# iamwangyabin/hardnetNas

Hardware: AMD Instinct MI355X
Metric: Mpatches/s (32×32→128-D) at 1/2/4/8 MI355X; HPatches FPR95 parity (higher is better)
Workload: dtype bf16x3; 1 GPU; Stock HardNet forward, 262144 synthetic 32x32 patches per GPU; model=hardnet, global_batch=262144, per_gpu_batch=262144, parallelism=dp1

## Files before the change

### hardnetnas_amd/csrc/hn_api.hip

```cpp
#include "hardnet_mi355x.h"
#include "hn_api_util.h"
#include "hn_internal.h"
#include "hn_pack.h"

#include <algorithm>
#include <atomic>
#include <cmath>
#include <cstdlib>
#include <cstring>
#include <map>
#include <mutex>
#include <string>
#include <utility>
#include <vector>

static thread_local std::string g_err;

static int env_int(const char* name, int dflt) {
  const char* e = std::getenv(name);
  return e ? std::atoi(e) : dflt;
}

void hn_read_knobs(HnKnobs* k) {
  *k = HnKnobs{};
// ... 2 lines not shown
  k->head_pf = env_int("HN_HEAD_PF", 1) != 0;
  k->fdl_valu = std::getenv("HN_FDL_VALU") != nullptr;
  k->naive_pw = std::getenv("HN_NAIVE_PW") != nullptr;
  k->naive_dw = std::getenv("HN_NAIVE_DW") != nullptr;
  k->no_skipfuse = std::getenv("HN_NO_SKIPFUSE") != nullptr;
  k->no_irfskip = std::getenv("HN_NO_IRFSKIP") != nullptr;
  k->pairdist_valu = std::getenv("HN_PAIRDIST_VALU") != nullptr;
  k->pairdist_reg = env_int("HN_PAIRDIST_REG", 0) != 0;
  k->pairdist_spread = env_int("HN_PAIRDIST_SPREAD", 1) != 0;
  k->front_fold = env_int("HN_FRONT_FOLD", 0) != 0;
  k->u8_apart = env_int("HN_U8_APART", 0) != 0;
  k->front_xch3 = env_int("HN_FRONT_XCH3", 0) != 0;
  k->no_mpfront = env_int("HN_NO_MPFRONT", 0) != 0;
  k->pipeline = env_int("HN_PIPELINE", 0) != 0;
  k->dyn_tiles = env_int("HN_STATIC_TILES", 0) != 0 ? 0 : env_int("HN_DYN_TILES", 3) & (kTilesConv3 | kTilesConv5);

  k->train_splitk = std::max(32, env_int("HN_TRAIN_SPLITK", 1024)) / 32 * 32;
  k->train_f32 = env_int("HN_TRAIN_F32", 17) & 255;
#ifdef HN_EXPERIMENTS
  k->c12_abl = env_int("HN_C12_ABL", 0) & 4095;
  k->c12w_pd = env_int("HN_C12W_PD", 11);
  k->dbg = env_int("HN_DEBUG", 0);
  k->head_abl = env_int("HN_HEAD_ABL", 0);
  k->w4_abl = env_int("HN_W4_ABL", 0);
  k->pairdist_abl = env_int("HN_PAIRDIST_ABL", 0);
  k->irf3 = env_int("HN_IRF3", 0) != 0;
#endif
}

static thread_local const HnKnobs* tl_knobs = nullptr;
// ... 286 lines not shown
    Folded f = fold(w, per, cout[l], nullptr, nullptr, mean, var, eps);
    int rc;
    if (l == 0) {
      std::vector<float> sw(9 * 32);
      for (int n = 0; n < 32; ++n)
        for (int t = 0; t < 9; ++t) sw[t * 32 + n] = f.w[n * 9 + t];
      if ((rc = m->upload(sw, &m->hd.stem_w))) return rc;
      if ((rc = m->upload(f.b, &m->hd.stem_b))) return rc;
      continue;
    }
    std::vector<uint16_t> pk = (l < 6) ? pack_conv3x3(f.w, cin[l], cout[l]) : pack_head(f.w, 128, 8);
    uint16_t* d = nullptr;
    if ((rc = m->upload(pk, &d))) return rc;
    m->hd.wpack[l] = d;
    if ((rc = m->upload(f.b, &m->hd.bias[l]))) return rc;
    if (l == 3 || l == 5) {
      uint16_t* c = nullptr;
      if ((rc = m->upload(pack_wino1(f.w, cin[l], cout[l]), &c))) return rc;
      m->hd.wino1[l] = c;
    }
#ifdef HN_EXPERIMENTS
    if (l == 3) {
      uint16_t* c = nullptr;
      if ((rc = m->upload(pack_wino4(f.w, cin[l], cout[l]), &c))) return rc;
      m->hd.wino4[l] = c;
    }
    if (l == 3 || l == 5) {
      uint16_t* c = nullptr;
      if ((rc = m->upload(pack_wino(f.w, cin[l], cout[l]), &c))) return rc;
      m->hd.wino[l] = c;
// ... 220 lines not shown
      if (*c >= '0' && *c <= '9') variant[i++] = *c - '0';
      else if (*c >= 'a' && *c <= 'z') variant[i++] = 10 + (*c - 'a');
  }
  hn_read_knobs(&m->knobs);
  if (m->knobs.head == 4 && !std::getenv("HN_CHUNK")) m->chunk = 65536;
  for (int l = 0; l < 6; ++l)
    if (!(m->conv[l] = hn_hardnet_conv_row(l, variant[l]))) {
      const std::string msg = "HN_VARIANT: tiling " + std::to_string(variant[l]) +
                              " is not available for layer " + std::to_string(l);
      delete m;
      return fail(HN_ERR_ARG, msg);
    }
  if (!hn_c12_cfg_ok(m->knobs.c12_cfg, m->knobs.c12_abl, m->knobs.c12w_pd)) {
    delete m;
    return fail(HN_ERR_ARG, "HN_C12_CFG / HN_C12_ABL / HN_C12W_PD: no such k_c12 build in this library");
  }
  if (m->knobs.head < 1 || m->knobs.head > 4) {
    delete m;
    return fail(HN_ERR_ARG, "HN_HEAD: head GEMM form must be 1, 2, 3 or 4");
  }
  (void)hipGetDevice(&m->device);
  Cursor cur{host_params, n_params};
  tl_f16_out_of_range = 0;
  rc = desc->kind == HN_KIND_HARDNET ? build_hardnet(m, cur)
       : desc->kind == HN_KIND_NAS    ? build_nas(m, cur)
                                      : build_fdl(m, cur);
  if (!rc && cur.i != n_params) rc = fail(HN_ERR_ARG, "host_params not fully consumed");
  if (!rc && tl_f16_out_of_range)
    rc = fail(HN_ERR_ARG, std::to_string(tl_f16_out_of_range) +
                              " BN-folded weights are outside the fp16 range of the fp16x3 kernels (|w| >= 65520 "
// ... 457 lines not shown
```

### hardnetnas_amd/csrc/hn_common.h

```cpp
#pragma once
#include <hip/hip_runtime.h>
#include <stdint.h>

typedef __bf16 bf16x8 __attribute__((ext_vector_type(8)));
typedef float f32x16 __attribute__((ext_vector_type(16)));
typedef float f32x4 __attribute__((ext_vector_type(4)));

#define HN_DEV __device__ __forceinline__

HN_DEV float relu0(float x) { return __builtin_bit_cast(float, __builtin_elementwise_max(__builtin_bit_cast(int, x), 0)); }
HN_DEV f32x4 relu4(f32x4 v) { return f32x4{relu0(v[0]), relu0(v[1]), relu0(v[2]), relu0(v[3])}; }

HN_DEV void split_bf16(float x, __bf16& hi, __bf16& lo) {
  hi = (__bf16)x;
  lo = (__bf16)(x - (float)hi);
}

typedef __bf16 bf16x4 __attribute__((ext_vector_type(4)));

HN_DEV void split8(const float4& a, const float4& b, uint4& hi, uint4& lo) {
  const float v[8] = {a.x, a.y, a.z, a.w, b.x, b.y, b.z, b.w};
  bf16x8 h, l;
#pragma unroll
  for (int j = 0; j < 8; ++j) {
// ... 46 lines not shown
                        f32x16 acc) {
  acc = __builtin_amdgcn_mfma_f32_32x32x16_f16(al, bh, acc, 0, 0, 0);
  acc = __builtin_amdgcn_mfma_f32_32x32x16_f16(ah, bl, acc, 0, 0, 0);
  acc = __builtin_amdgcn_mfma_f32_32x32x16_f16(ah, bh, acc, 0, 0, 0);
  return acc;
}

typedef float f32x4_t __attribute__((ext_vector_type(4)));
HN_DEV f32x4_t mfma3_f16_16(const f16x8& ah, const f16x8& al, const f16x8& bh, const f16x8& bl, f32x4_t acc) {
  acc = __builtin_amdgcn_mfma_f32_16x16x32_f16(al, bh, acc, 0, 0, 0);
  acc = __builtin_amdgcn_mfma_f32_16x16x32_f16(ah, bl, acc, 0, 0, 0);
  acc = __builtin_amdgcn_mfma_f32_16x16x32_f16(ah, bh, acc, 0, 0, 0);
  return acc;
}

HN_DEV int xcd_remap(int bid, int nblocks) {
  const int xcd = bid & 7, idx = bid >> 3;
  const int q = nblocks >> 3, r = nblocks & 7;
  return (xcd < r ? xcd * (q + 1) : r * (q + 1) + (xcd - r) * q) + idx;
}

HN_DEV float wave_sum(float v) {
#pragma unroll
  for (int o = 32; o > 0; o >>= 1) v += __shfl_xor(v, o, 64);
  return v;
}

HN_DEV float half_sum(float v) {
#pragma unroll
  for (int o = 16; o > 0; o >>= 1) v += __shfl_xor(v, o, 64);
// ... 3 lines not shown
```

### hardnetnas_amd/csrc/hn_hardnet.hip

```cpp
#include "hn_common.h"
#include "hn_internal.h"

#include <algorithm>
#include <cstdlib>

template <bool NORM>
__global__ __launch_bounds__(256) void k_stem(const float* __restrict__ in, float* __restrict__ out,
                                              const float* __restrict__ w,
                                              const float* __restrict__ b,
                                              float eps) {
  __shared__ float tile[34 * 34];
  __shared__ float red[8];
  const int t = threadIdx.x;
  const size_t p = blockIdx.x;
  const float4 v = reinterpret_cast<const float4*>(in + p * 1024)[t];
  for (int i = t; i < 34 * 34; i += 256) tile[i] = 0.f;
  float mean = 0.f, sd = 1.f;
  if (NORM) {
    float s = wave_sum(v.x + v.y + v.z + v.w);
    if ((t & 63) == 0) red[t >> 6] = s;
    __syncthreads();
    mean = (red[0] + red[1] + red[2] + red[3]) * (1.f / 1024.f);
    const float d0 = v.x - mean, d1 = v.y - mean, d2 = v.z - mean, d3 = v.w - mean;
    float q = wave_sum(d0 * d0 + d1 * d1 + d2 * d2 + d3 * d3);
// ... 633 lines not shown
  static constexpr int SCR = 32 * SROW * 4;
  static constexpr int OSTR = COUT * 4 + 16;
  static constexpr int OCH = B::BM * COUT / 4;
  static constexpr int OPT = OCH / PTHR;
  static constexpr int MB = PST ? (B::BM < BUF / OSTR ? B::BM : BUF / OSTR) : 0;
  static constexpr int XST = PST ? (B::BM - MB) * OSTR : 0;
  static constexpr int BIAS_OFF = 2 * BUF + (STEM ? NWP * PBUF : 0) + (CST ? NWC * SCR : 0);
  static constexpr int SMEM = BIAS_OFF + COUT * 4 + XST;
  static constexpr bool DEEP = !STEM && UPT <= 6;
  static_assert(SMEM <= 160 * 1024, "LDS");
  static_assert(!(STEM && CST), "the CST epilogue scratch starts where the STEM buffers live");
  static_assert(!PST || (!STEM && !CST && OCH % PTHR == 0), "PST");
};

template <int CIN, int COUT, int HIN, int S, int NP, int TR, int WM, int WN, bool STEM, int ABL = 0,
          int PX = 80, bool CST = false, bool PST = false>
__global__ __launch_bounds__((WM * WN + 4) * 64) void k_conv_ws(
    const float* __restrict__ in, float* __restrict__ out, const uint4* __restrict__ wp,
    const float* __restrict__ bias, int P, const float* __restrict__ stem_w,
    const float* __restrict__ stem_b, float eps, float relu_lo) {
  using C = WsCfg<CIN, COUT, HIN, S, NP, TR, WM, WN, STEM, PX, CST, PST>;
  static_assert(PX == 80 || !STEM, "the stem producer writes the 80-byte layout");
  extern __shared__ __attribute__((aligned(16))) char smem[];
  const int tid = threadIdx.x, lane = tid & 63;
  const int wave = __builtin_amdgcn_readfirstlane(tid >> 6);
  const bool producer = wave >= C::NWC;
  const int r = lane & 31, h = lane >> 5;
  const int nwg = gridDim.x, rb = xcd_remap(blockIdx.x, nwg);
  const int ntiles = (P + NP - 1) / NP * C::RT;
  const int per = (ntiles + nwg - 1) / nwg;
  const int t_begin = STEM ? rb * per : rb;
// ... 160 lines not shown
#pragma unroll
        for (int q = 0; q < 4; ++q) {
          bf16x4 oh, ol;
#pragma unroll
          for (int j = 0; j < 4; ++j) {
            const float v = inside ? fmaxf(c0[4 * q + j] + b16[4 * q + j], 0.f) : 0.f;
            oh[j] = (__bf16)v;
            ol[j] = (__bf16)(v - (float)oh[j]);
          }
          *reinterpret_cast<uint2*>(o + 16 * q) = __builtin_bit_cast(uint2, oh);
          *reinterpret_cast<uint2*>(o + C::PLANE + 16 * q) = __builtin_bit_cast(uint2, ol);
        }
      }
    }
  };

  if (producer) {
    if constexpr (STEM) {
      static_assert(CIN == 32 && HIN == 32 && S == 1 && NP == 1, "stem fusion is conv1-only");
      for (int i = lane; i < 34 * 34; i += 64) pt[i] = 0.f;
      stem_loads(0);
      stem_write(0, buf0);
    } else {
      produce_loads(0, pf);
      produce_write(buf0, pf);
      if (NS > 1) produce_loads(1, pf);
    }
  } else {
    for (int i = tid; i < COUT; i += C::NWC * 64) reinterpret_cast<float*>(smem + C::BIAS_OFF)[i] = bias[i];
  }
// ... 781 lines not shown

using Conv1s = Direct<32, 32, 32, 1, 1, 8, 4, 1, true>;
using Conv1 = Direct<32, 32, 32, 1, 1, 8, 4, 1, false>;
using Conv2 = Direct<32, 64, 32, 2, 1, 8, 2, 2, false>;
using Conv3 = Direct<64, 64, 16, 1, 1, 16, 2, 2, false>;
using Conv4 = Direct<64, 128, 16, 2, 1, 8, 1, 4, false>;
using Conv5 = Direct<128, 128, 8, 1, 2, 8, 1, 4, false>;
using Pipe5Cst = Pipe<128, 128, 8, 1, 2, 8, 1, 4, false, 0, true>;
using Ws1s = Ws<32, 32, 32, 1, 1, 4, 4, 1, true, 0, 80, false, false>;
using Ws1sT8 = Ws<32, 32, 32, 1, 1, 8, 4, 1, true, 0, 80, false, false>;
using Ws2 = Ws<32, 64, 32, 2, 1, 4, 2, 2, false, 0, 80, false, false>;
using Ws2T2 = Ws<32, 64, 32, 2, 1, 2, 1, 2, false, 0, 80, false, false>;
using Ws4Np2 = Ws<64, 128, 16, 2, 2, 8, 2, 2, false, 0, 64, false, false>;
using Ws4Pst = Ws<64, 128, 16, 2, 2, 8, 2, 2, false, 0, 64, false, true>;
using Ws3Cst = Ws<64, 64, 16, 1, 1, 16, 2, 2, false, 0, 80, true, false>;

constexpr HnConvRow kConvRows[] = {
    {0, 0, row<0, Conv1s>},
    {0, 5, row<0, Ws1s>},
    {0, 6, row<0, Ws1sT8>},
    {1, 0, row<1, Conv1>},
    {1, 5, row<1, Conv1>},
    {1, 6, row<1, Conv1>},
    {2, 0, row<2, Conv2>},
    {2, 5, row<2, Ws2>},
    {2, 6, row<2, Ws2T2>},
    {3, 0, row<3, Conv3>},
    {3, 16, row<3, Ws3Cst>},
    {4, 0, row<4, Conv4>},
    {4, 15, row<4, Ws4Np2>},
    {4, 18, row<4, Ws4Pst>},
    {5, 0, row<5, Conv5>},
    {5, 16, row<5, Pipe5Cst>},
#ifdef HN_EXPERIMENTS
    {0, 1, row<0, Direct<32, 32, 32, 1, 1, 4, 4, 1, true>>},
    {2, 1, row<2, Direct<32, 64, 32, 2, 1, 4, 2, 2, false>>},
    {3, 1, row<3, Direct<64, 64, 16, 1, 1, 8, 2, 2, false>>},
    {4, 1, row<4, Direct<64, 128, 16, 2, 1, 4, 1, 4, false>>},
    {5, 1, row<5, Direct<128, 128, 8, 1, 1, 8, 1, 4, false>>},
    {0, 2, row<0, Pipe<32, 32, 32, 1, 1, 4, 4, 1, true, 0, false>>},
    {0, 3, row<0, Pipe<32, 32, 32, 1, 1, 8, 4, 1, true, 0, false>>},
    {2, 2, row<2, Pipe<32, 64, 32, 2, 1, 2, 1, 2, false, 0, false>>},
    {2, 3, row<2, Pipe<32, 64, 32, 2, 1, 4, 2, 2, false, 0, false>>},
    {3, 2, row<3, Pipe<64, 64, 16, 1, 1, 8, 2, 2, false, 0, false>>},
    {3, 3, row<3, Pipe<64, 64, 16, 1, 1, 16, 2, 2, false, 0, false>>},
    {4, 2, row<4, Pipe<64, 128, 16, 2, 1, 4, 1, 4, false, 0, false>>},
// ... 144 lines not shown
```

### hardnetnas_amd/csrc/hn_internal.h

```cpp
#pragma once
#include <hip/hip_runtime.h>

#include <algorithm>
#include <type_traits>

#include "hardnet_mi355x.h"

struct HnKnobs {
  int c12_cfg = 15;
  int head = 4;
  bool head_pf = true;
  bool fdl_valu = false;
  bool naive_pw = false;
  bool naive_dw = false;
  bool no_skipfuse = false;
  bool no_irfskip = false;
  bool pairdist_valu = false;
  bool pairdist_reg = false;
  bool pairdist_spread = true;
  bool front_fold = false;
  bool u8_apart = false;
  bool front_xch3 = false;
  bool no_mpfront = false;
  bool pipeline = false;
  bool irf3 = false;
  int dyn_tiles = 3;
  int train_splitk = 1024;
  int train_f32 = 17;
  int c12w_pd = 11;
  int c12_abl = 0;
  int head_abl = 0;
  int w4_abl = 0;
  int pairdist_abl = 0;
  int dbg = 0;
};
void hn_read_knobs(HnKnobs* k);
const HnKnobs& hn_knobs();

constexpr int kTilesConv3 = 1, kTilesConv5 = 2;
constexpr int kTileLaunches = 32;
unsigned* hn_tile_counters(int kernel);

hipError_t hn_resident_blocks(const void* fn, int nthreads, int lds, int* resident);

struct HardnetDev {
  float* stem_w = nullptr;
  float* stem_b = nullptr;
  void* wpack[7] = {};
  float* bias[7] = {};
  void* c12_w1 = nullptr;
  void* c12_w2 = nullptr;
  void* c12_w1w = nullptr;
  void* wino[7] = {};
  void* wino1[7] = {};
  void* wino4[7] = {};
};
struct HnU8In {
  const uint8_t* in;
  int resize;
  int normalize;
  float mean, stdv;
};
hipError_t hn_launch_c12(const float* in, float* out, const HardnetDev& d, int P, float eps,
                         hipStream_t st, const HnU8In* u8 = nullptr);

hipError_t hn_launch_stem(const float* in, float* out, const float* w, const float* b, int P,
                          bool norm, float eps, hipStream_t st);
using HnConvLaunch = hipError_t (*)(const HardnetDev& d, const float* in, float* out, int P, float eps,
                                    hipStream_t st);
// ... 278 lines not shown
```

### hardnetnas_amd/csrc/hn_pack.h

```cpp
#pragma once
#include <cmath>
#include <cstddef>
#include <cstdint>
#include <cstring>
#include <vector>

namespace {

uint16_t f2bf(float x) {
  uint32_t u;
  std::memcpy(&u, &x, 4);
  u += 0x7FFFu + ((u >> 16) & 1u);
  return (uint16_t)(u >> 16);
}
float bf2f(uint16_t b) {
  uint32_t u = (uint32_t)b << 16;
  float f;
  std::memcpy(&f, &u, 4);
  return f;
}

struct Folded {
  std::vector<float> w, b;
};
// ... 25 lines not shown
          uint16_t* lo = &out[o + 64 * 8];
          for (int lane = 0; lane < 64; ++lane)
            for (int j = 0; j < 8; ++j) {
              const int n = nt * 32 + (lane & 31);
              const int c = cc * 32 + ks * 16 + (lane >> 5) * 8 + j;
              const float v = w[((size_t)n * cin + c) * 9 + tap];
              const uint16_t h = f2bf(v);
              hi[lane * 8 + j] = h;
              lo[lane * 8 + j] = f2bf(v - bf2f(h));
            }
          o += 2 * 64 * 8;
        }
  return out;
}

static thread_local long tl_f16_out_of_range = 0;
static void put_f16_split(float v, uint16_t* hi, uint16_t* lo) {
  const _Float16 hv = (_Float16)v;
  if (!std::isfinite((float)hv)) ++tl_f16_out_of_range;
  const _Float16 lv = (_Float16)(v - (float)hv);
  std::memcpy(hi, &hv, 2);
  std::memcpy(lo, &lv, 2);
}

static std::vector<uint16_t> pack_head(const std::vector<float>& w, int cin, int kk, bool f16 = false) {
  const int K = cin * kk * kk;
  std::vector<uint16_t> out((size_t)(K / 16) * 4 * 2 * 64 * 8);
  size_t o = 0;
  for (int ks = 0; ks < K / 16; ++ks)
    for (int nt = 0; nt < 4; ++nt) {
// ... 145 lines not shown
          for (int j = 0; j < 8; ++j) {
            const int n = nt * 32 + (lane & 31);
            const int c = cc * 32 + ks * 16 + (lane >> 5) * 8 + j;
            double u = 0;
            for (int t = 0; t < 3; ++t) u += G[xi][t] * (double)w[((size_t)n * cin + c) * 9 + ky * 3 + t];
            const float v = (float)(xi == 3 ? -u : u);
            const uint16_t hv = f2bf(v);
            hi[lane * 8 + j] = hv;
            lo[lane * 8 + j] = f2bf(v - bf2f(hv));
          }
        o += 2 * 64 * 8;
      }
  return out;
}

static std::vector<uint16_t> pack_wino4(const std::vector<float>& w, int cin, int cout) {
  static const double G[6][3] = {{4, 0, 0},
                                 {2.0 / 3, 2.0 / 3, 2.0 / 3},
                                 {2.0 / 3, -2.0 / 3, 2.0 / 3},
                                 {-8.0 / 3, -4.0 / 3, -2.0 / 3},
                                 {-8.0 / 3, 4.0 / 3, -2.0 / 3},
                                 {0, 0, 1}};
  static const int XO[6] = {0, 5, 1, 2, 3, 4};
  const int ncc = cin / 32, ntot = cout / 16;
  std::vector<uint16_t> out((size_t)ncc * 18 * ntot * 2 * 64 * 8);
  size_t o = 0;
  for (int cc = 0; cc < ncc; ++cc)
    for (int kx = 0; kx < 18; ++kx)
      for (int nt = 0; nt < ntot; ++nt) {
        const int xi = XO[kx / 3], ky = kx % 3;
// ... 51 lines not shown
```

### hardnetnas_amd/csrc/hn_wino1.hip

```cpp
#include "hn_common.h"
#include "hn_internal.h"
#include "hn_tiles.h"

namespace {

template <int CIN, int COUT, int H, int NP, int WM, int WN, bool CST>
struct W1Cfg {
  static constexpr int TR = H;
  static constexpr int NTX = H / 2;
  static constexpr int BM = NP * TR * NTX;
  static constexpr int MT = BM / WM / 32, NT = COUT / WN / 32;
  static constexpr int NTOT = COUT / 32, NCC = CIN / 32;
  static constexpr int XROW = NTX * 64;
  static constexpr int RS = 4 * XROW;
  static constexpr int PS = TR * RS;
  static constexpr int ZROW = NP * PS;
  static constexpr int PLANE = ZROW + RS;
  static constexpr int BUF = 2 * PLANE;
  static constexpr int NWC = WM * WN, NWP = 4, NTHR = (NWC + NWP) * 64, PTHR = NWP * 64;
  static constexpr int UNITS = NP * TR * NTX * 4;
  static_assert(64 % (4 * NTX) == 0 && PTHR % (4 * NTX) == 0, "a row's units share one wave");
  static constexpr int UPT = (UNITS + PTHR - 1) / PTHR;
  static constexpr bool DEEP = UPT <= 2;
  static constexpr int SROW = 36;
// ... 16 lines not shown
}
template <int N, class F>
HN_DEV void static_for(F&& f) {
  static_for_seq(std::make_integer_sequence<int, N>{}, f);
}

constexpr int w1_lo3(int g) { return g == 0 ? 0 : g == 1 ? 6 : g == 2 ? 11 : 16; }
constexpr int w1_fold_valu(bool first, int kx, int g) {
  if (kx == 11 && g >= 3) return 2 * (w1_lo3(g - 2) - w1_lo3(g - 3));
  if (kx == 12 && g < 3) return 2 * (w1_lo3(g + 1) - w1_lo3(g));
  if (kx == 18 || kx == 19 || (kx == 0 && !first)) return g < 5 ? 3 : 1;
  if (kx == 23 && g >= 3) return w1_lo3(g - 2) - w1_lo3(g - 3);
  return 0;
}

template <int CIN, int COUT, int H, int NP, int WM, int WN, bool CST, int WD = 3, int ABL = 0, bool DYN = false>
__global__ __launch_bounds__((WM * WN + 4) * 64) void k_conv_w1(const float* __restrict__ in, float* __restrict__ out,
                                                                const uint4* __restrict__ wp,
                                                                const float* __restrict__ bias, int P,
                                                                unsigned* __restrict__ tile_ctr,
                                                                long long* __restrict__ stamps) {
  using C = W1Cfg<CIN, COUT, H, NP, WM, WN, CST>;
  static_assert(!DYN || ((ABL & ~256) == 0 && C::DEEP && C::NCC % 2 == 0),
                "claimed tiles: the two-stage producer body, whole bodies per tile, no ablation");
  constexpr int TR = C::TR;
  extern __shared__ __attribute__((aligned(16))) char smem[];
  const int tid = threadIdx.x, lane = tid & 63;
  const int wave = __builtin_amdgcn_readfirstlane(tid >> 6);
  const bool producer = wave >= C::NWC;
  const int r = lane & 31, h = lane >> 5;
  const int nwg = gridDim.x, rb = xcd_remap(blockIdx.x, nwg);
// ... 149 lines not shown
        __syncthreads();
        if (s + 1 >= NS) break;
        produce_loads(s + 3, pf);
        produce_write(buf0, pf2);
        __syncthreads();
      }
    }
    return;
  }

  for (int i = tid; i < COUT; i += C::NWC * 64) reinterpret_cast<float*>(smem + C::BIAS_OFF)[i] = bias[i];
  __syncthreads();
  if constexpr ((ABL & 16) != 0) {
#pragma unroll 1
    for (int s = 0; s < NS; ++s) __syncthreads();
    return;
  }
  const int wm = wave / WN, wn = wave % WN;
  const float* const sbias = reinterpret_cast<const float*>(smem + C::BIAS_OFF);
  int ylr[C::MT], vo[C::MT][3][2];
#pragma unroll
  for (int mt = 0; mt < C::MT; ++mt) {
    const int m = (wm * C::MT + mt) * 32 + r;
    const int np = m / (TR * C::NTX), rem = m % (TR * C::NTX);
    ylr[mt] = rem / C::NTX;
#pragma unroll
    for (int ky = 0; ky < 3; ++ky) {
      const int wr = ylr[mt] + ky;
      const int rowb = (wr >= 1 && wr <= TR) ? np * C::PS + (wr - 1) * C::RS : C::ZROW;
#pragma unroll
// ... 179 lines not shown
  }
  if constexpr ((ABL & 256) != 0) {
    if (tid == 0) stamps[2 * blockIdx.x + 1] = (long long)__builtin_amdgcn_s_memrealtime();
  }
}

template <int L, int CIN, int COUT, int H, int NP, int WM, int WN, bool CST, int WD, int ABL>
hipError_t launch_w1(const HardnetDev& d, const float* in, float* out, int P, float, hipStream_t st) {
  using C = W1Cfg<CIN, COUT, H, NP, WM, WN, CST>;
  if (!d.wino1[L]) return hipErrorInvalidValue;
  const uint4* w = static_cast<const uint4*>(d.wino1[L]);
  long long* stamps = nullptr;
  if constexpr ((ABL & 256) != 0)
    stamps = reinterpret_cast<long long*>((L == 3 ? out + (size_t)P * 40960 : const_cast<float*>(in) + (size_t)P * 24576) +
                                          (2 << 20) / 4) + (L == 3 ? 0 : 2048);
  if constexpr ((ABL & ~256) == 0) {
    if (unsigned* ctr = hn_tile_counters(L == 3 ? kTilesConv3 : kTilesConv5))
      return hn_launch_persistent<&k_conv_w1<CIN, COUT, H, NP, WM, WN, CST, WD, ABL, true>, C::NTHR, C::SMEM>(
          (P + NP - 1) / NP, st, in, out, w, d.bias[L], P, ctr, stamps);
  }
  return hn_launch_persistent<&k_conv_w1<CIN, COUT, H, NP, WM, WN, CST, WD, ABL>, C::NTHR, C::SMEM>(
      (P + NP - 1) / NP, st, in, out, w, d.bias[L], P, (unsigned*)nullptr, stamps);
}

#ifdef HN_EXPERIMENTS
template <int CIN, int COUT, int H, int NP, int WN>
struct W4Cfg {
  static constexpr int NTX = H / 4;
  static constexpr int POS = NP * H * NTX;
  static constexpr int MT = POS / 16;
// ... 376 lines not shown
```

Before: 5.543 Mpatches/s.

## Use 16x16x32 bf16 MFMA path for conv4 with repacked weights

Adds a conv4 consumer path that uses the 16x16x32 bf16 MFMA instruction instead of the 32x32 form. Conv4 weights are repacked into a 16-row fragment layout, and A/B fragments are loaded on a 3-deep weight ring. The path is on by default through the HN_MFMA16 mask. Equivalent 16-wide Winograd variants for conv3 and conv5 exist only in the experiments build. The aim is better MFMA issue efficiency and register use in conv4. The cost is an extra packed weight buffer and a new hand-scheduled kernel body that has to keep bf16x3 accuracy.

```diff
diff --git a/hardnetnas_amd/csrc/hn_api.hip b/hardnetnas_amd/csrc/hn_api.hip
--- a/hardnetnas_amd/csrc/hn_api.hip
+++ b/hardnetnas_amd/csrc/hn_api.hip
@@ -40,6 +40,7 @@
   k->no_mpfront = env_int("HN_NO_MPFRONT", 0) != 0;
   k->pipeline = env_int("HN_PIPELINE", 0) != 0;
   k->dyn_tiles = env_int("HN_STATIC_TILES", 0) != 0 ? 0 : env_int("HN_DYN_TILES", 3) & (kTilesConv3 | kTilesConv5);
+  k->mfma16 = env_int("HN_MFMA16", kMfma16Conv4);
 
   k->train_splitk = std::max(32, env_int("HN_TRAIN_SPLITK", 1024)) / 32 * 32;
   k->train_f32 = env_int("HN_TRAIN_F32", 17) & 255;
@@ -356,6 +357,18 @@
     if ((rc = m->upload(pk, &d))) return rc;
     m->hd.wpack[l] = d;
     if ((rc = m->upload(f.b, &m->hd.bias[l]))) return rc;
+    if (l == 4 && (m->knobs.mfma16 & kMfma16Conv4)) {
+      uint16_t* c = nullptr;
+      if ((rc = m->upload(pack_conv3x3_16(f.w, cin[l], cout[l]), &c))) return rc;
+      m->hd.wpack16[l] = c;
+    }
+#ifdef HN_EXPERIMENTS
+    if ((l == 3 && (m->knobs.mfma16 & kMfma16Conv3)) || (l == 5 && (m->knobs.mfma16 & kMfma16Conv5))) {
+      uint16_t* c = nullptr;
+      if ((rc = m->upload(pack_wino1_16(f.w, cin[l], cout[l], l == 5), &c))) return rc;
+      m->hd.wino1_16[l] = c;
+    }
+#endif
     if (l == 3 || l == 5) {
       uint16_t* c = nullptr;
       if ((rc = m->upload(pack_wino1(f.w, cin[l], cout[l]), &c))) return rc;
@@ -606,6 +619,10 @@
   if (!hn_c12_cfg_ok(m->knobs.c12_cfg, m->knobs.c12_abl, m->knobs.c12w_pd)) {
     delete m;
     return fail(HN_ERR_ARG, "HN_C12_CFG / HN_C12_ABL / HN_C12W_PD: no such k_c12 build in this library");
+  }
+  if (m->knobs.mfma16 & ~kMfma16Built) {
+    delete m;
+    return fail(HN_ERR_ARG, "HN_MFMA16: a mask of 2 (conv4); 1 (conv3) and 4 (conv5) in the experiments library only");
   }
   if (m->knobs.head < 1 || m->knobs.head > 4) {
     delete m;
diff --git a/hardnetnas_amd/csrc/hn_common.h b/hardnetnas_amd/csrc/hn_common.h
--- a/hardnetnas_amd/csrc/hn_common.h
+++ b/hardnetnas_amd/csrc/hn_common.h
@@ -84,6 +84,10 @@
   return acc;
 }
 
+HN_DEV f32x4_t mfma16(const bf16x8& a, const bf16x8& b, f32x4_t acc) {
+  return __builtin_amdgcn_mfma_f32_16x16x32_bf16(a, b, acc, 0, 0, 0);
+}
+
 HN_DEV int xcd_remap(int bid, int nblocks) {
   const int xcd = bid & 7, idx = bid >> 3;
   const int q = nblocks >> 3, r = nblocks & 7;
diff --git a/hardnetnas_amd/csrc/hn_hardnet.hip b/hardnetnas_amd/csrc/hn_hardnet.hip
--- a/hardnetnas_amd/csrc/hn_hardnet.hip
+++ b/hardnetnas_amd/csrc/hn_hardnet.hip
@@ -671,7 +671,7 @@
 };
 
 template <int CIN, int COUT, int HIN, int S, int NP, int TR, int WM, int WN, bool STEM, int ABL = 0,
-          int PX = 80, bool CST = false, bool PST = false>
+          int PX = 80, bool CST = false, bool PST = false, bool S16 = false>
 __global__ __launch_bounds__((WM * WN + 4) * 64) void k_conv_ws(
     const float* __restrict__ in, float* __restrict__ out, const uint4* __restrict__ wp,
     const float* __restrict__ bias, int P, const float* __restrict__ stem_w,
@@ -862,6 +862,140 @@
       }
     }
   };
+
+  if constexpr (S16) {
+    static_assert(PX == 64 && S == 2 && C::MT == 2 && C::NT == 2 && C::WOUT == 8 && !STEM && !CST && ABL == 0,
+                  "S16: conv4's two-patch tiling on the swizzled window");
+    if (!producer) {
+      for (int i = tid; i < COUT; i += C::NWC * 64) reinterpret_cast<float*>(smem + C::BIAS_OFF)[i] = bias[i];
+      __syncthreads();
+      const int wm = wave / WN, wn = wave % WN;
+      const float* const sbias = reinterpret_cast<const float*>(smem + C::BIAS_OFF);
+      const int kq = lane >> 4;
+      int abv[4][2], mrow[4];
+#pragma unroll
+      for (int pg = 0; pg < 4; ++pg) {
+        const int m = (wm * C::MT + (pg >> 1)) * 32 + (lane & 7) + 8 * (pg & 1) + 16 * ((lane >> 3) & 1);
+        const int np = m / (TR * C::WOUT), rem = m % (TR * C::WOUT);
+        const int yl = rem / C::WOUT, xo = rem % C::WOUT;
+#pragma unroll
+        for (int v = 0; v < 2; ++v) abv[pg][v] = np * C::PS + yl * S * C::RS + xo * PX + 16 * (kq ^ ((yl + v) & 3));
+        mrow[pg] = m;
+      }
+      static_assert(C::PLANE + 2 * C::RS + C::colofs(1) * PX + 16 < 65536, "a tap's offset is an immediate");
+      constexpr unsigned GROUP_BYTES = 2 * 64 * 16, STEP_BYTES = (COUT / 16) * GROUP_BYTES;
+      constexpr unsigned CHUNK_BYTES = 9 * STEP_BYTES;
+      const __amdgpu_buffer_rsrc_t wr_ = make_rsrc(wp, C::NCC * CHUNK_BYTES);
+      const unsigned wvoff = wn * 4 * GROUP_BYTES + lane * 16;
+      constexpr int NH = 18;
+      constexpr int WD = 3;
+      static_assert(NH % WD == 0, "the weight ring runs on across stages");
+      auto load_b = [&](int cc, int hx, uint4 (&dst)[2][2]) {
+#pragma unroll
+        for (int cg = 0; cg < 2; ++cg) {
+          const unsigned k = cc * CHUNK_BYTES + (hx >> 1) * STEP_BYTES + (2 * (hx & 1) + cg) * GROUP_BYTES;
+          dst[cg][0] = buf_load16(wr_, wvoff, k);
+          dst[cg][1] = buf_load16(wr_, wvoff, k + 64 * 16);
+        }
+      };
+      uint4 bq[WD][2][2];
+#pragma unroll
+      for (int k = 0; k + 1 < WD; ++k) load_b(0, k, bq[k]);
+      f32x4_t acc[4][4];
+      auto stage = [&](auto first, int s, int cc, int ccn) {
+        constexpr bool FIRST = decltype(first)::value;
+        const char* cur = (s & 1) ? buf1 : buf0;
+        uint4 aq[4][2];
+        const char* ap[4][2];
+#pragma unroll
+        for (int pg = 0; pg < 4; ++pg) {
+          ap[pg][0] = cur + abv[pg][0];
+          ap[pg][1] = cur + abv[pg][1];
+        }
+        auto load_a = [&](int tap, int pg) {
+          const int toff = (tap / 3) * C::RS + C::colofs(tap % 3) * PX;
+          const char* a = ap[pg][(tap / 3) / S];
+          aq[pg][0] = *reinterpret_cast<const uint4*>(a + toff);
+          aq[pg][1] = *reinterpret_cast<const uint4*>(a + C::PLANE + toff);
+        };
+#pragma unroll
+        for (int pg = 0; pg < 4; ++pg) load_a(0, pg);
+#pragma unroll
+        for (int hx = 0; hx < NH; ++hx) {
+          const int tap = hx >> 1, ch = hx & 1;
+          if (hx + WD - 1 < NH)
+            load_b(cc, hx + WD - 1, bq[(hx + WD - 1) % WD]);
+          else
+            load_b(ccn, hx + WD - 1 - NH, bq[(hx + WD - 1) % WD]);
+          __builtin_amdgcn_sched_barrier(0);
+          if constexpr (PST) {
+            if (FIRST && hx == 0 && s > 0) __builtin_amdgcn_s_barrier();
+          }
+          const bf16x8 w0h = as_bf16x8(bq[hx % WD][0][0]), w0l = as_bf16x8(bq[hx % WD][0][1]);
+          const bf16x8 w1h = as_bf16x8(bq[hx % WD][1][0]), w1l = as_bf16x8(bq[hx % WD][1][1]);
+#pragma unroll
+          for (int pg = 0; pg < 4; ++pg) {
+            const bf16x8 xh = as_bf16x8(aq[pg][0]), xl = as_bf16x8(aq[pg][1]);
+            f32x4_t c0 = FIRST && tap == 0 ? f32x4_t{} : acc[pg][2 * ch];
+            f32x4_t c1 = FIRST && tap == 0 ? f32x4_t{} : acc[pg][2 * ch + 1];
+            c0 = mfma16(w0l, xh, c0);
+            c1 = mfma16(w1l, xh, c1);
+            c0 = mfma16(w0h, xl, c0);
+            c1 = mfma16(w1h, xl, c1);
+            c0 = mfma16(w0h, xh, c0);
+            c1 = mfma16(w1h, xh, c1);
+            acc[pg][2 * ch] = c0;
+            acc[pg][2 * ch + 1] = c1;
+            __builtin_amdgcn_sched_barrier(0);
+            if (ch == 1 && tap + 1 < 9) {
+              load_a(tap + 1, pg);
+              __builtin_amdgcn_sched_barrier(0);
+            }
+          }
+          __builtin_amdgcn_sched_barrier(0);
+        }
+      };
+#pragma unroll 1
+      for (int t = 0; t < my_tiles; ++t) {
+        const int s0 = t * C::NCC, s = s0 + C::NCC - 1;
+        stage(std::true_type{}, s0, 0, C::NCC > 1 ? 1 : 0);
+#pragma unroll 1
+        for (int cc = 1; cc < C::NCC; ++cc) {
+          __syncthreads();
+          stage(std::false_type{}, s0 + cc, cc, (cc + 1) % C::NCC);
+        }
+        int p0 = 0, y0 = 0;
+        char* stg = (s & 1) ? buf1 : buf0;
+        if constexpr (PST)
+          __syncthreads();
+        else
+          tile_of(s, p0, y0);
+#pragma unroll
+        for (int cg = 0; cg < 4; ++cg) {
+          const int ch0 = wn * C::NT * 32 + 16 * cg + 4 * kq;
+          const float4 bv = *reinterpret_cast<const float4*>(sbias + ch0);
+#pragma unroll
+          for (int pg = 0; pg < 4; ++pg) {
+            float4 v;
+            v.x = fmaxf(acc[pg][cg][0] + bv.x, relu_lo);
+            v.y = fmaxf(acc[pg][cg][1] + bv.y, relu_lo);
+            v.z = fmaxf(acc[pg][cg][2] + bv.z, relu_lo);
+            v.w = fmaxf(acc[pg][cg][3] + bv.w, relu_lo);
+            if constexpr (PST) {
+              *reinterpret_cast<float4*>(stage_at(stg, mrow[pg]) + ch0 * 4) = v;
+            } else {
+              const bool ok = NP == 1 || p0 + ((wm * C::MT + (pg >> 1)) * 32) / (TR * C::WOUT) < P;
+              if (ok)
+                *reinterpret_cast<float4*>(out + ((size_t)(p0 * C::HOUT + y0) * C::WOUT + mrow[pg]) * COUT + ch0) = v;
+            }
+          }
+        }
+        __syncthreads();
+      }
+      if constexpr (PST) __builtin_amdgcn_s_barrier();
+      return;
+    }
+  }
 
   if (producer) {
     if constexpr (STEM) {
@@ -1673,6 +1807,15 @@
 using Ws4Np2 = Ws<64, 128, 16, 2, 2, 8, 2, 2, false, 0, 64, false, false>;
 using Ws4Pst = Ws<64, 128, 16, 2, 2, 8, 2, 2, false, 0, 64, false, true>;
 using Ws3Cst = Ws<64, 64, 16, 1, 1, 16, 2, 2, false, 0, 80, true, false>;
+template <bool PST>
+using Ws4S16 = ConvBuild<&k_conv_ws<64, 128, 16, 2, 2, 8, 2, 2, false, 0, 64, false, PST, true>,
+                         WsCfg<64, 128, 16, 2, 2, 8, 2, 2, false, 64, false, PST>, 2, false, true>;
+template <class B, class B16>
+hipError_t row4(const HardnetDev& d, const float* in, float* out, int P, float eps, hipStream_t st) {
+  if (d.wpack16[4])
+    return conv_launch<B16>(in, out, d.wpack16[4], d.bias[4], P, nullptr, nullptr, 0.f, st, 0.f);
+  return row<4, B>(d, in, out, P, eps, st);
+}
 
 constexpr HnConvRow kConvRows[] = {
     {0, 0, row<0, Conv1s>},
@@ -1687,8 +1830,8 @@
     {3, 0, row<3, Conv3>},
     {3, 16, row<3, Ws3Cst>},
     {4, 0, row<4, Conv4>},
-    {4, 15, row<4, Ws4Np2>},
-    {4, 18, row<4, Ws4Pst>},
+    {4, 15, row4<Ws4Np2, Ws4S16<false>>},
+    {4, 18, row4<Ws4Pst, Ws4S16<true>>},
     {5, 0, row<5, Conv5>},
     {5, 16, row<5, Pipe5Cst>},
 #ifdef HN_EXPERIMENTS
diff --git a/hardnetnas_amd/csrc/hn_internal.h b/hardnetnas_amd/csrc/hn_internal.h
--- a/hardnetnas_amd/csrc/hn_internal.h
+++ b/hardnetnas_amd/csrc/hn_internal.h
@@ -25,6 +25,7 @@
   bool pipeline = false;
   bool irf3 = false;
   int dyn_tiles = 3;
+  int mfma16 = 2;
   int train_splitk = 1024;
   int train_f32 = 17;
   int c12w_pd = 11;
@@ -39,6 +40,12 @@
 
 constexpr int kTilesConv3 = 1, kTilesConv5 = 2;
 constexpr int kTileLaunches = 32;
+constexpr int kMfma16Conv3 = 1, kMfma16Conv4 = 2, kMfma16Conv5 = 4;
+#ifdef HN_EXPERIMENTS
+constexpr int kMfma16Built = kMfma16Conv3 | kMfma16Conv4 | kMfma16Conv5;
+#else
+constexpr int kMfma16Built = kMfma16Conv4;
+#endif
 unsigned* hn_tile_counters(int kernel);
 
 hipError_t hn_resident_blocks(const void* fn, int nthreads, int lds, int* resident);
@@ -47,12 +54,14 @@
   float* stem_w = nullptr;
   float* stem_b = nullptr;
   void* wpack[7] = {};
+  void* wpack16[7] = {};
   float* bias[7] = {};
   void* c12_w1 = nullptr;
   void* c12_w2 = nullptr;
   void* c12_w1w = nullptr;
   void* wino[7] = {};
   void* wino1[7] = {};
+  void* wino1_16[7] = {};
   void* wino4[7] = {};
 };
 struct HnU8In {
diff --git a/hardnetnas_amd/csrc/hn_pack.h b/hardnetnas_amd/csrc/hn_pack.h
--- a/hardnetnas_amd/csrc/hn_pack.h
+++ b/hardnetnas_amd/csrc/hn_pack.h
@@ -63,6 +63,29 @@
   return out;
 }
 
+static std::vector<uint16_t> pack_conv3x3_16(const std::vector<float>& w, int cin, int cout) {
+  const int ncc = cin / 32, ng = cout / 16;
+  std::vector<uint16_t> out((size_t)ncc * 9 * ng * 2 * 64 * 8);
+  size_t o = 0;
+  for (int cc = 0; cc < ncc; ++cc)
+    for (int tap = 0; tap < 9; ++tap)
+      for (int g = 0; g < ng; ++g) {
+        uint16_t* hi = &out[o];
+        uint16_t* lo = &out[o + 64 * 8];
+        for (int lane = 0; lane < 64; ++lane)
+          for (int j = 0; j < 8; ++j) {
+            const int n = g * 16 + (lane & 15);
+            const int c = cc * 32 + (lane >> 4) * 8 + j;
+            const float v = w[((size_t)n * cin + c) * 9 + tap];
+            const uint16_t h = f2bf(v);
+            hi[lane * 8 + j] = h;
+            lo[lane * 8 + j] = f2bf(v - bf2f(h));
+          }
+        o += 2 * 64 * 8;
+      }
+  return out;
+}
+
 static thread_local long tl_f16_out_of_range = 0;
 static void put_f16_split(float v, uint16_t* hi, uint16_t* lo) {
   const _Float16 hv = (_Float16)v;
@@ -238,6 +261,36 @@
   return out;
 }
 
+#ifdef HN_EXPERIMENTS
+static std::vector<uint16_t> pack_wino1_16(const std::vector<float>& w, int cin, int cout, bool swap12) {
+  static const double G[4][3] = {{1, 0, 0}, {0.5, 0.5, 0.5}, {0.5, -0.5, 0.5}, {0, 0, 1}};
+  const int ncc = cin / 32, ng = cout / 16;
+  std::vector<uint16_t> out((size_t)ncc * 12 * ng * 2 * 64 * 8);
+  size_t o = 0;
+  for (int cc = 0; cc < ncc; ++cc)
+    for (int sx = 0; sx < 12; ++sx)
+      for (int g = 0; g < ng; ++g) {
+        const int xi = sx / 3, ky = sx % 3;
+        uint16_t* hi = &out[o];
+        uint16_t* lo = &out[o + 64 * 8];
+        for (int lane = 0; lane < 64; ++lane)
+          for (int j = 0; j < 8; ++j) {
+            const int q = lane >> 4, kq = swap12 && (q == 1 || q == 2) ? 3 - q : q;
+            const int n = g * 16 + (lane & 15);
+            const int c = cc * 32 + kq * 8 + j;
+            double u = 0;
+            for (int t = 0; t < 3; ++t) u += G[xi][t] * (double)w[((size_t)n * cin + c) * 9 + ky * 3 + t];
+            const float v = (float)(xi == 3 ? -u : u);
+            const uint16_t hv = f2bf(v);
+            hi[lane * 8 + j] = hv;
+            lo[lane * 8 + j] = f2bf(v - bf2f(hv));
+          }
+        o += 2 * 64 * 8;
+      }
+  return out;
+}
+#endif
+
 static std::vector<uint16_t> pack_wino4(const std::vector<float>& w, int cin, int cout) {
   static const double G[6][3] = {{4, 0, 0},
                                  {2.0 / 3, 2.0 / 3, 2.0 / 3},
diff --git a/hardnetnas_amd/csrc/hn_pack16_host_check.cpp b/hardnetnas_amd/csrc/hn_pack16_host_check.cpp
--- /dev/null
+++ b/hardnetnas_amd/csrc/hn_pack16_host_check.cpp
@@ -0,0 +1,158 @@
+#include <cinttypes>
+#include <cstdio>
+#include <cstdlib>
+#include <fstream>
+#include <map>
+#include <sstream>
+#include <string>
+
+#include "hn_pack.h"
+
+namespace pack16check {
+
+#define CHECK(cond, ...)                          \
+  do {                                            \
+    if (!(cond)) {                                \
+      std::fprintf(stderr, "FAILED %s: ", #cond); \
+      std::fprintf(stderr, __VA_ARGS__);          \
+      std::fprintf(stderr, "\n");                 \
+      std::exit(1);                               \
+    }                                             \
+  } while (0)
+
+constexpr uint64_t kFnvBasis = 0xcbf29ce484222325ull, kFnvPrime = 0x100000001b3ull;
+uint64_t fnv1a(const std::vector<uint16_t>& v) {
+  uint64_t h = kFnvBasis;
+  const unsigned char* p = reinterpret_cast<const unsigned char*>(v.data());
+  for (size_t i = 0; i < v.size() * sizeof(uint16_t); ++i) h = (h ^ p[i]) * kFnvPrime;
+  return h;
+}
+
+std::vector<float> weights(const std::string& key, size_t n) {
+  uint64_t s = kFnvBasis;
+  for (unsigned char c : key) s = (s ^ c) * kFnvPrime;
+  std::vector<float> w(n);
+  for (float& x : w) {
+    s = s * 6364136223846793005ull + 1442695040888963407ull;
+    x = (float)((double)(s >> 40) / (double)(1 << 23) - 1.0);
+  }
+  return w;
+}
+
+constexpr size_t kFrag = 2 * 64 * 8;
+
+void dump(const std::string& dir, const char* packer, int cin, int cout, const std::vector<uint16_t>& v) {
+  const std::string path = dir + "/" + packer + "_" + std::to_string(cin) + "_" + std::to_string(cout) + ".u16";
+  std::ofstream f(path, std::ios::binary);
+  f.write(reinterpret_cast<const char*>(v.data()), (std::streamsize)(v.size() * sizeof(uint16_t)));
+  CHECK(f.good(), "cannot write %s", path.c_str());
+}
+
+uint64_t conv3x3_16(int cin, int cout, const std::string& dump_dir) {
+  const std::string key = "pack_conv3x3_16 " + std::to_string(cin) + "," + std::to_string(cout);
+  const std::vector<float> w = weights(key, (size_t)cout * cin * 9);
+  const std::vector<uint16_t> a = pack_conv3x3_16(w, cin, cout), ref = pack_conv3x3(w, cin, cout);
+  const size_t want = (size_t)(cin / 32) * 9 * (cout / 16) * kFrag;
+  CHECK(a.size() == want, "%s: %zu elements, the layout has %zu", key.c_str(), a.size(), want);
+  CHECK(a.size() == ref.size(), "%s: %zu elements, pack_conv3x3 has %zu", key.c_str(), a.size(), ref.size());
+  bool written = false;
+  for (size_t i = want - kFrag; i < want; ++i) written |= a[i] != 0;
+  CHECK(written, "%s: the write cursor stopped before the end of the output", key.c_str());
+  std::vector<int> seen((size_t)cout * cin * 9, 0);
+  const int ng = cout / 16, ntot = cout / 32;
+  for (int cc = 0; cc < cin / 32; ++cc)
+    for (int tap = 0; tap < 9; ++tap)
+      for (int g = 0; g < ng; ++g)
+        for (int lane = 0; lane < 64; ++lane)
+          for (int j = 0; j < 8; ++j) {
+            const int n = 16 * g + (lane & 15), cl = 8 * (lane >> 4) + j;
+            const size_t o = (((size_t)(cc * 9 + tap) * ng + g) * 2 * 64 + lane) * 8 + j;
+            const int ks = cl / 16, rl = (n & 31) + 32 * ((cl % 16) / 8);
+            const size_t r = (((((size_t)(cc * 9 + tap) * 2 + ks) * ntot + n / 32) * 2) * 64 + rl) * 8 + j;
+            CHECK(a[o] == ref[r] && a[o + 64 * 8] == ref[r + 64 * 8],
+                  "%s: (n %d, c %d, tap %d) differs from pack_conv3x3", key.c_str(), n, 32 * cc + cl, tap);
+            ++seen[((size_t)n * cin + 32 * cc + cl) * 9 + tap];
+          }
+  for (int s : seen) CHECK(s == 1, "%s: an (output channel, input channel, tap) written %d times", key.c_str(), s);
+  if (!dump_dir.empty()) {
+    dump(dump_dir, "pack_conv3x3_16", cin, cout, a);
+    dump(dump_dir, "pack_conv3x3", cin, cout, ref);
+  }
+  return fnv1a(a);
+}
+
+uint64_t wino1_16(int cin, int cout, bool swap12, const std::string& dump_dir) {
+  const std::string key =
+      "pack_wino1_16 " + std::to_string(cin) + "," + std::to_string(cout) + "," + (swap12 ? "1" : "0");
+  const std::vector<float> w = weights(key, (size_t)cout * cin * 9);
+  const std::vector<uint16_t> a = pack_wino1_16(w, cin, cout, swap12), ref = pack_wino1(w, cin, cout);
+  const size_t want = (size_t)(cin / 32) * 12 * (cout / 16) * kFrag;
+  CHECK(a.size() == want, "%s: %zu elements, the layout has %zu", key.c_str(), a.size(), want);
+  CHECK(a.size() == ref.size(), "%s: %zu elements, pack_wino1 has %zu", key.c_str(), a.size(), ref.size());
+  bool written = false;
+  for (size_t i = want - kFrag; i < want; ++i) written |= a[i] != 0;
+  CHECK(written, "%s: the write cursor stopped before the end of the output", key.c_str());
+  std::vector<int> seen((size_t)cout * cin * 12, 0);
+  const int ng = cout / 16, ntot = cout / 32;
+  for (int cc = 0; cc < cin / 32; ++cc)
+    for (int sx = 0; sx < 12; ++sx)
+      for (int g = 0; g < ng; ++g)
+        for (int lane = 0; lane < 64; ++lane)
+          for (int j = 0; j < 8; ++j) {
+            const int q = lane >> 4, kq = swap12 && (q == 1 || q == 2) ? 3 - q : q;
+            const int n = 16 * g + (lane & 15), cl = 8 * kq + j;
+            const size_t o = (((size_t)(cc * 12 + sx) * ng + g) * 2 * 64 + lane) * 8 + j;
+            const int kx = 6 * (sx / 3) + 2 * (sx % 3) + cl / 16, rl = (n & 31) + 32 * ((cl % 16) / 8);
+            const size_t r = ((((size_t)(cc * 24 + kx) * ntot + n / 32) * 2) * 64 + rl) * 8 + j;
+            CHECK(a[o] == ref[r] && a[o + 64 * 8] == ref[r + 64 * 8],
+                  "%s: (n %d, c %d, step %d) differs from pack_wino1", key.c_str(), n, 32 * cc + cl, sx);
+            ++seen[((size_t)n * cin + 32 * cc + cl) * 12 + sx];
+          }
+  for (int s : seen) CHECK(s == 1, "%s: an (output channel, input channel, step) written %d times", key.c_str(), s);
+  if (!dump_dir.empty()) {
+    dump(dump_dir, "pack_wino1_16", cin, cout, a);
+    dump(dump_dir, "pack_wino1", cin, cout, ref);
+  }
+  return fnv1a(a);
+}
+
+}
+
+int main(int argc, char** argv) {
+  using namespace pack16check;
+  if (argc < 2 || argc > 3) {
+    std::fprintf(stderr, "usage: %s tests/golden/pack16_digests.txt | --print | --dump DIR\n", argv[0]);
+    return 2;
+  }
+  const std::string mode = argv[1];
+  CHECK((mode == "--dump") == (argc == 3), "--dump takes a directory, the other modes no argument");
+  std::map<std::string, uint64_t> done;
+  const std::string dir = mode == "--dump" ? argv[2] : "";
+  done["pack_conv3x3_16 64,128"] = conv3x3_16(64, 128, dir);
+  done["pack_wino1_16 64,64,0"] = wino1_16(64, 64, false, dir);
+  done["pack_wino1_16 128,128,1"] = wino1_16(128, 128, true, dir);
+  if (mode == "--dump") return 0;
+  if (mode == "--print") {
+    for (const auto& kv : done) std::printf("%s %016" PRIx64 "\n", kv.first.c_str(), kv.second);
+    return 0;
+  }
+  std::ifstream f(argv[1]);
+  CHECK(f.good(), "cannot read %s", argv[1]);
+  std::map<std::string, uint64_t> golden;
+  for (std::string line; std::getline(f, line);) {
+    if (line.empty() || line[0] == '#') continue;
+    std::istringstream s(line);
+    std::string packer, shape, digest;
+    CHECK(bool(s >> packer >> shape >> digest), "%s: malformed line '%s'", argv[1], line.c_str());
+    golden[packer + " " + shape] = std::strtoull(digest.c_str(), nullptr, 16);
+  }
+  for (const auto& kv : done) {
+    CHECK(golden.count(kv.first), "%s has no line for '%s'", argv[1], kv.first.c_str());
+    CHECK(golden[kv.first] == kv.second, "%s: digest %016" PRIx64 ", recorded %016" PRIx64, kv.first.c_str(), kv.second,
+          golden[kv.first]);
+  }
+  CHECK(golden.size() == done.size(), "%s has %zu lines, the packer is called at %zu shapes", argv[1], golden.size(),
+        done.size());
+  std::printf("pack16_check: %zu (packer, shape) pairs, sizes, elements and digests match\n", done.size());
+  return 0;
+}
diff --git a/hardnetnas_amd/csrc/hn_wino1.hip b/hardnetnas_amd/csrc/hn_wino1.hip
--- a/hardnetnas_amd/csrc/hn_wino1.hip
+++ b/hardnetnas_amd/csrc/hn_wino1.hip
@@ -54,7 +54,194 @@
   return 0;
 }
 
-template <int CIN, int COUT, int H, int NP, int WM, int WN, bool CST, int WD = 3, int ABL = 0, bool DYN = false>
+constexpr int w1_lo12(int g) { return 16 * g / 12; }
+constexpr int w1_fold16_valu(bool first, int hx, int g) {
+  const int n = w1_lo12(g + 1) - w1_lo12(g);
+  if (hx == 11 || hx == 12) return 2 * n;
+  if (hx == 17 || hx == 18 || hx == 23 || (hx == 0 && !first)) return n;
+  return 0;
+}
+template <class C, int COUT, int H, int NP, int WN, int WD, bool DYN, class TileOf>
+HN_DEV void w1_mfma16(char* smem, char* buf0, char* buf1, int* tq, float* __restrict__ out,
+                      const uint4* __restrict__ wp, int P, int wave, int lane, int my_tiles, TileOf tile_of) {
+  constexpr int TR = C::TR, WS = WD / 2, NSX = 12, NHX = 24;
+  static_assert(C::MT == 2 && C::NT == 1 && WD % 2 == 0 && NSX % WS == 0, "S16: two M tiles x one N tile per wave");
+  constexpr bool SWAP12 = C::NTX == 4;
+  const int wm = wave / WN, wn = wave % WN;
+  const float* const sbias = reinterpret_cast<const float*>(smem + C::BIAS_OFF);
+  auto pos = [&](int l, int pgl) { return (l & 7) + 8 * pgl + 16 * ((l >> 3) & 1); };
+  int vo[4][3];
+  {
+    const int kq = lane >> 4, kc = SWAP12 && (kq == 1 || kq == 2) ? 3 - kq : kq;
+#pragma unroll
+    for (int pg = 0; pg < 4; ++pg) {
+      const int m = (wm * C::MT + (pg >> 1)) * 32 + pos(lane, pg & 1);
+      const int np = m / (TR * C::NTX), rem = m % (TR * C::NTX), yl = rem / C::NTX;
+#pragma unroll
+      for (int ky = 0; ky < 3; ++ky) {
+        const int wr = yl + ky;
+        const int rowb = (wr >= 1 && wr <= TR) ? np * C::PS + (wr - 1) * C::RS : C::ZROW;
+        vo[pg][ky] = rowb + (rem % C::NTX) * 64 + 16 * (kc ^ (wr & 3));
+        asm volatile("" : "+v"(vo[pg][ky]));
+      }
+    }
+  }
+  constexpr unsigned GROUP_BYTES = 2 * 64 * 16, STEP_BYTES = (COUT / 16) * GROUP_BYTES;
+  static_assert(NSX * STEP_BYTES == C::CHUNK_BYTES, "the same bytes as pack_wino1");
+  const __amdgpu_buffer_rsrc_t wr_ = make_rsrc(wp, C::NCC * C::CHUNK_BYTES);
+  const unsigned wvoff = wn * 2 * GROUP_BYTES + lane * 16;
+  auto load_b = [&](int cc, int sx, uint4 (&dst)[2][2]) {
+#pragma unroll
+    for (int cg = 0; cg < 2; ++cg) {
+      const unsigned k = cc * C::CHUNK_BYTES + sx * STEP_BYTES + cg * GROUP_BYTES;
+      dst[cg][0] = buf_load16(wr_, wvoff, k);
+      dst[cg][1] = buf_load16(wr_, wvoff, k + 64 * 16);
+    }
+  };
+  uint4 bq[WS][2][2];
+#pragma unroll
+  for (int k = 0; k + 1 < WS; ++k) load_b(0, k, bq[k]);
+  f32x4_t y0a[4][2], y1a[4][2], ma[4][2];
+  auto sadd = [](float a, float b) {
+    float v = a + b;
+    asm("" : "+v"(v));
+    return v;
+  };
+  auto ssub = [](float a, float b) {
+    float v = a - b;
+    asm("" : "+v"(v));
+    return v;
+  };
+#define W1E(a, j, e) a[2 * (j) + ((e) >> 3)][((e) >> 2) & 1][(e) & 3]
+  auto fold = [&](auto first_, auto hx_, auto g_) {
+    constexpr bool first = decltype(first_)::value;
+    constexpr int hx = decltype(hx_)::value, g = decltype(g_)::value;
+#pragma unroll
+    for (int e = w1_lo12(g); e < w1_lo12(g + 1); ++e) {
+      if constexpr (hx == 11 || hx == 12) {
+        constexpr int j = hx - 11;
+        W1E(y0a, j, e) = sadd(W1E(y0a, j, e), W1E(ma, j, e));
+        W1E(y1a, j, e) = sadd(first ? 0.f : W1E(y1a, j, e), W1E(ma, j, e));
+      } else if constexpr (hx == 17 || hx == 18) {
+        constexpr int j = hx - 17;
+        W1E(y0a, j, e) = sadd(W1E(y0a, j, e), W1E(ma, j, e));
+      } else if constexpr (hx == 23) {
+        W1E(y1a, 0, e) = ssub(W1E(y1a, 0, e), W1E(ma, 0, e));
+      } else if constexpr (hx == 0 && !first) {
+        W1E(y1a, 1, e) = ssub(W1E(y1a, 1, e), W1E(ma, 1, e));
+      }
+    }
+  };
+  auto stage = [&](auto first_, int s, int cc, int ccn) {
+    constexpr bool FIRST = decltype(first_)::value;
+    const char* cur = (s & 1) ? buf1 : buf0;
+    uint4 aq[2][2][2];
+    auto load_a = [&](int hx, uint4 (&dst)[2][2]) {
+      const int sx = hx >> 1, mt = hx & 1, xi = sx / 3, ky = sx % 3;
+#pragma unroll
+      for (int pgl = 0; pgl < 2; ++pgl) {
+        const char* pa = cur + vo[2 * mt + pgl][ky];
+        dst[pgl][0] = *reinterpret_cast<const uint4*>(pa + xi * C::XROW);
+        dst[pgl][1] = *reinterpret_cast<const uint4*>(pa + (C::PLANE + xi * C::XROW));
+      }
+    };
+    load_a(0, aq[0]);
+    static_for<NHX>([&](auto hx_) {
+      constexpr int hx = decltype(hx_)::value, sx = hx >> 1, mt = hx & 1, xi = sx / 3;
+      if constexpr (mt == 0) {
+        if constexpr (sx + WS - 1 < NSX)
+          load_b(cc, sx + WS - 1, bq[(sx + WS - 1) % WS]);
+        else
+          load_b(ccn, sx + WS - 1 - NSX, bq[(sx + WS - 1) % WS]);
+      }
+      if constexpr (hx + 1 < NHX) load_a(hx + 1, aq[(hx + 1) & 1]);
+      __builtin_amdgcn_sched_barrier(0);
+      static_for<12>([&](auto g_) {
+        constexpr int g = decltype(g_)::value, pgl = g / 6, cg = g & 1, p = (g % 6) >> 1, pg = 2 * mt + pgl;
+        const bf16x8 x = as_bf16x8(aq[hx & 1][pgl][p == 1 ? 1 : 0]), w = as_bf16x8(bq[sx % WS][cg][p == 0 ? 1 : 0]);
+        f32x4_t& acc = xi == 0 ? y0a[pg][cg] : xi == 3 ? y1a[pg][cg] : ma[pg][cg];
+        constexpr bool zero = p == 0 && (sx == 3 || sx == 6 || (sx == 0 && FIRST));
+        acc = mfma16(w, x, zero ? f32x4_t{} : acc);
+        constexpr int nv = w1_fold16_valu(FIRST, hx, g);
+        if constexpr (nv > 0) {
+          fold(first_, hx_, g_);
+          __builtin_amdgcn_sched_group_barrier(0x008, 1, 0);
+          __builtin_amdgcn_sched_group_barrier(0x002, nv, 0);
+        } else if constexpr (w1_fold16_valu(FIRST, hx, 1) > 0) {
+          __builtin_amdgcn_sched_group_barrier(0x008, 1, 0);
+        }
+      });
+      __builtin_amdgcn_sched_barrier(0);
+    });
+  };
+  hn_tiles::Cursor c{0, 0, 0};
+  if constexpr (DYN) {
+    hn_tiles::cursor_start(c, tq);
+    c.cur = __builtin_amdgcn_readfirstlane(c.cur);
+  }
+#pragma unroll 1
+  for (int t = 0; DYN ? !hn_tiles::cursor_done(c) : t < my_tiles; ++t) {
+    const int s0 = DYN ? 0 : t * C::NCC, s = s0 + C::NCC - 1;
+    stage(std::true_type{}, s0, 0, C::NCC > 1 ? 1 : 0);
+#pragma unroll 1
+    for (int cc = 1; cc < C::NCC; ++cc) {
+      __syncthreads();
+      stage(std::false_type{}, s0 + cc, cc, (cc + 1) % C::NCC);
+    }
+#pragma unroll
+    for (int e = 0; e < 16; ++e) W1E(y1a, 1, e) = ssub(W1E(y1a, 1, e), W1E(ma, 1, e));
+    {
+      const int p0 = DYN ? c.cur * NP : tile_of(s);
+      int le = lane;
+      asm volatile("" : "+v"(le));
+      const int kq = le >> 4;
+      float4 bv[2];
+#pragma unroll
+      for (int cg = 0; cg < 2; ++cg) bv[cg] = *reinterpret_cast<const float4*>(sbias + wn * 32 + 16 * cg + 4 * kq);
+#pragma unroll
+      for (int mt = 0; mt < C::MT; ++mt) {
+        const int m0 = (wm * C::MT + mt) * 32;
+        const int np = m0 / (TR * C::NTX), yb = (m0 % (TR * C::NTX)) / C::NTX;
+        if (NP == 1 || p0 + np < P) {
+          float* const ob = out + (((size_t)p0 + np) * H + yb) * H * COUT + wn * 32;
+#pragma unroll
+          for (int par = 0; par < 2; ++par) {
+            float* scr = reinterpret_cast<float*>(smem + C::SCR_OFF) + wave * (C::SCR / 4);
+#pragma unroll
+            for (int pgl = 0; pgl < 2; ++pgl)
+#pragma unroll
+              for (int cg = 0; cg < 2; ++cg) {
+                const f32x4_t yv = par ? y1a[2 * mt + pgl][cg] : y0a[2 * mt + pgl][cg];
+                const float4 v = make_float4(relu0(yv[0] + bv[cg].x), relu0(yv[1] + bv[cg].y),
+                                             relu0(yv[2] + bv[cg].z), relu0(yv[3] + bv[cg].w));
+                *reinterpret_cast<float4*>(scr + pos(le, pgl) * C::SROW + 16 * cg + 4 * kq) = v;
+              }
+            __builtin_amdgcn_wave_barrier();
+            asm volatile("" ::: "memory");
+#pragma unroll
+            for (int k = 0; k < 4; ++k) {
+              const int ml = 8 * k + (le >> 3), c4 = le & 7;
+              const int px = (ml / C::NTX) * H + 2 * (ml % C::NTX) + par;
+              *reinterpret_cast<float4*>(ob + (size_t)px * COUT + 4 * c4) =
+                  *reinterpret_cast<const float4*>(scr + ml * C::SROW + 4 * c4);
+            }
+            __builtin_amdgcn_wave_barrier();
+            asm volatile("" ::: "memory");
+          }
+        }
+      }
+    }
+    __syncthreads();
+    if constexpr (DYN) {
+      hn_tiles::cursor_advance(c, tq);
+      c.cur = __builtin_amdgcn_readfirstlane(c.cur);
+    }
+  }
+#undef W1E
+}
+
+template <int CIN, int COUT, int H, int NP, int WM, int WN, bool CST, int WD = 3, int ABL = 0, bool DYN = false,
+          bool S16 = false>
 __global__ __launch_bounds__((WM * WN + 4) * 64) void k_conv_w1(const float* __restrict__ in, float* __restrict__ out,
                                                                 const uint4* __restrict__ wp,
                                                                 const float* __restrict__ bias, int P,
@@ -234,6 +421,12 @@
   if constexpr ((ABL & 16) != 0) {
 #pragma unroll 1
     for (int s = 0; s < NS; ++s) __syncthreads();
+    return;
+  }
+  if constexpr (S16) {
+    static_assert(CST && ABL == 0, "S16: the production rows' form");
+    w1_mfma16<C, COUT, H, NP, WN, WD, DYN>(smem, buf0, buf1, tq, out, wp, P, wave, lane, my_tiles,
+                                           [&](int s) { return tile_of(s); });
     return;
   }
   const int wm = wave / WN, wn = wave % WN;
@@ -443,6 +636,17 @@
   if constexpr ((ABL & 256) != 0)
     stamps = reinterpret_cast<long long*>((L == 3 ? out + (size_t)P * 40960 : const_cast<float*>(in) + (size_t)P * 24576) +
                                           (2 << 20) / 4) + (L == 3 ? 0 : 2048);
+#ifdef HN_EXPERIMENTS
+  if constexpr (ABL == 0 && CST && WD % 2 == 0) {
+    if (const uint4* w16 = static_cast<const uint4*>(d.wino1_16[L])) {
+      if (unsigned* ctr = hn_tile_counters(L == 3 ? kTilesConv3 : kTilesConv5))
+        return hn_launch_persistent<&k_conv_w1<CIN, COUT, H, NP, WM, WN, CST, WD, 0, true, true>, C::NTHR, C::SMEM>(
+            (P + NP - 1) / NP, st, in, out, w16, d.bias[L], P, ctr, stamps);
+      return hn_launch_persistent<&k_conv_w1<CIN, COUT, H, NP, WM, WN, CST, WD, 0, false, true>, C::NTHR, C::SMEM>(
+          (P + NP - 1) / NP, st, in, out, w16, d.bias[L], P, (unsigned*)nullptr, stamps);
+    }
+  }
+#endif
   if constexpr ((ABL & ~256) == 0) {
     if (unsigned* ctr = hn_tile_counters(L == 3 ? kTilesConv3 : kTilesConv5))
       return hn_launch_persistent<&k_conv_w1<CIN, COUT, H, NP, WM, WN, CST, WD, ABL, true>, C::NTHR, C::SMEM>(
```

After: 5.599 Mpatches/s (median of 6 runs). 1.0% higher.
